# zabaras/deep-turbulence

Measured on AMD Instinct MI355X. Metric: flow-field samples/sec (fwd+log-det+bwd), 64x256x256x4; optimizer step: HipAdam (one-launch Adam, same update as torch.optim.Adam), higher is better.
Workload: dtype f32; 1 GPU; tmglow M: sample()+logdet+backward+Adam, out 256x256x4, L=4, K=16, batch 64/GPU; global_batch=64, parallelism=dp1, world_size_observed=1, rank0_device=AMD Radeon Graphics cuda:0, mix_precision=f32, launch=eager

## Files before the change

### deep-turbulence_amd/csrc/tmg_conv.hip

```cpp
#include "tmg_common.h"
#include <stdlib.h>

static __device__ float g_tmg_zero_page[64];

struct ConvP {
    TmgSeg in[TMG_MAX_IN_SEG];
    int nseg;
    int vec4;
    int B, Hin, Win, Hout, Wout;
    int ksize, stride;
    int Cin, Cin_pad, Cout, Cout_pad;
    const float* wpk;
    const float* bias;
    const float* kappa;
    const float* in_scale;
    const float* in_shift;
    int relu_in, pad_rep, relu_out, accumulate;
    TmgOSeg out[TMG_MAX_OUT_SEG];
    int nout;
    TmgSeg add;
    int TW_log2, TH;
    int KCH;
    int tiles_x, tiles_y;
    int ntiles, nchunks;
    int ovec4;
};

template <int MT, int NTW, int WM, int WN>
__global__ __launch_bounds__(256) void conv_mfma_kernel(ConvP p) {
    extern __shared__ __attribute__((aligned(16))) float lds[];
    const int tid = threadIdx.x, lane = tid & 63, wave = tid >> 6;
    const int wm = wave % WM, wn = wave / WM;
    const int li = lane & 15, q = lane >> 4;
    constexpr int MBLK = 16 * MT * WM;

    int t = blockIdx.x;
    const int tx = t % p.tiles_x;
    t /= p.tiles_x;
    const int ty = t % p.tiles_y;
    const int b = t / p.tiles_y;
    const int TWl = p.TW_log2, TW = 1 << TWl, TH = MBLK >> TWl;
    const int oy0 = ty * TH, ox0 = tx * TW;
    const int s = p.stride, halo = p.ksize >> 1;
    const int PW = s * (TW - 1) + 1 + 2 * halo, PH = s * (TH - 1) + 1 + 2 * halo;
    const int iy0 = s * oy0 - halo, ix0 = s * ox0 - halo;
    const int ntaps = p.ksize * p.ksize;
    const int KB = p.Cin_pad >> 4;

// ... 97 lines not shown
        }
        float* obase = op_ + ooff + nl;
#pragma unroll
        for (int i = 0; i < MT; ++i) {
#pragma unroll
            for (int r = 0; r < 4; ++r) {
                const int m = (wm * MT + i) * 16 + q * 4 + r;
                const int oy = oy0 + (m >> TWl), ox = ox0 + (m & (TW - 1));
                if (oy < p.Hout && ox < p.Wout) {
                    const size_t opx = ((size_t)b * p.Hout + oy) * p.Wout + ox;
                    float v = acc[i][j][r] + bv;
                    if (p.add.p) v += p.add.p[opx * p.add.stride + p.add.off + n];
                    v *= osc;
                    if (p.relu_out) v = fmaxf(v, 0.f);
                    float* dst = obase + opx * ostride;
                    if (p.accumulate) v += *dst;
                    *dst = v;
                }
            }
        }
    }
}

template <int MT, int NTW, int WM, int WN>
__global__ __launch_bounds__(512, 1) void conv_fwd_kernel(ConvP p) {
    extern __shared__ __attribute__((aligned(16))) float lds[];
    constexpr int NT = 512, UP = 7;
    const int tid = threadIdx.x, lane = tid & 63;
    const int wave = __builtin_amdgcn_readfirstlane(tid >> 6);
    const int wm = wave % WM, wn = wave / WM;
    const int li = lane & 15, q = lane >> 4;
    constexpr int MBLK = 16 * MT * WM;
    const int TWl = p.TW_log2, TW = 1 << TWl, TH = MBLK >> TWl;
    const int halo = p.ksize >> 1, ntaps = p.ksize * p.ksize;
    const int PW = TW + 2 * halo, PH = TH + 2 * halo, PHPW = PH * PW;
    const int KB = p.Cin_pad >> 4, KCH = p.KCH, CS = KCH + 8, CS4 = CS >> 2;
    const int bufw = PHPW * CS;
    const int nchunks = p.nchunks;
    const int ntiles_total = p.Cout_pad >> 4;
    const int ntile0 = (blockIdx.y * WN + wn) * NTW;
    const float* zero_page = g_tmg_zero_page;

    f32x4 acc[MT][NTW];
#pragma unroll
    for (int i = 0; i < MT; ++i)
#pragma unroll
        for (int j = 0; j < NTW; ++j) acc[i][j] = (f32x4){0.f, 0.f, 0.f, 0.f};
    int abase[MT], mrc[MT];
// ... 31 lines not shown
    int ti_b = (int)blockIdx.x / tpi, ti_y = ((int)blockIdx.x - ti_b * tpi) / p.tiles_x, ti_x = (int)blockIdx.x - ti_b * tpi - ti_y * p.tiles_x;
    int tm_b = ti_b, tm_y = ti_y, tm_x = ti_x;
#define TMG_FW_ADVANCE(X, Y, B_)                                  \
    {                                                             \
        X += Gx;                                                  \
        if (X >= p.tiles_x) { X -= p.tiles_x; ++Y; }              \
        Y += Gy;                                                  \
        if (Y >= p.tiles_y) { Y -= p.tiles_y; ++B_; }             \
        B_ += Gb;                                                 \
    }
    const float osc = out_scale_of(p.kappa);
    constexpr bool HB = MT * NTW <= 8;
    float4 biasq[HB ? NTW : 1];
    if (HB) {
#pragma unroll
        for (int j = 0; j < NTW; ++j) {
            const int n0 = (ntile0 + j) * 16 + 4 * q;
            float b4[4];
#pragma unroll
            for (int r = 0; r < 4; ++r) b4[r] = (p.bias && n0 + r < p.Cout) ? p.bias[n0 + r] : 0.f;
            biasq[HB ? j : 0] = make_float4(b4[0], b4[1], b4[2], b4[3]);
        }
    }
    float4 b0[NTW], b1[NTW];
    if (nst > 0) {
#pragma unroll
        for (int j = 0; j < NTW; ++j) b0[j] = tmg_bload4(wrs, boff0, TMG_FW_BOFF(j));
    }

    for (int k = -2; k < nst; ++k) {
        if (k >= -1 && k + 1 < nst) {
            const int c0 = cc * KCH, kch = min(KCH, p.Cin_pad - c0);
            const bool pcv = 4 * pc4 < kch;
            float4 isc = make_float4(1.f, 1.f, 1.f, 1.f), ish = make_float4(0.f, 0.f, 0.f, 0.f);
            if (p.in_scale) {
                const int c = c0 + 4 * pc4;
                float* fs = reinterpret_cast<float*>(&isc);
                float* fh = reinterpret_cast<float*>(&ish);
#pragma unroll
                for (int e = 0; e < 4; ++e)
                    if (c + e < p.Cin) { fs[e] = p.in_scale[c + e]; fh[e] = p.in_shift[c + e]; }
            }
            char* bb = reinterpret_cast<char*>(lds) + 4u * (((k + 1) & 1) * bufw) + pdst0;
#pragma unroll
            for (int u = 0; u < UP; ++u) {
                if (pcv && ppix0 + u * pstep < PHPW) {
// ... 24 lines not shown
                        if (cl >= p.in[1].n) {
                            cl -= p.in[1].n;
                            sp = p.in[2].p; ss = p.in[2].stride; so = p.in[2].off;
                        }
                    }
                    tptr = sp + so + cl;
                    tss = ss;
                }
            }
            const int iy0 = oy0_ - halo, ix0 = ox0_ - halo;
            const int tbv = b_ * p.Hin * p.Win * tss;
            oobm = 0;
#pragma unroll
            for (int u = 0; u < UP; ++u) {
                const int iy = iy0 + (int)(pyx[u] >> 16), ix = ix0 + (int)(pyx[u] & 0xffffu);
                const int iyc = min(max(iy, 0), p.Hin - 1), ixc = min(max(ix, 0), p.Win - 1);
                const bool oob = !p.pad_rep && (iy != iyc || ix != ixc);
                const int elem = (int)__umul24(__umul24(iyc, p.Win) + ixc, tss) + tbv;
                const float* a_ = (oob || ppix0 + u * pstep >= PHPW) ? zero_page : tptr + elem;
                pv[u] = *reinterpret_cast<const float4*>(a_);
                if (p.in_scale) oobm |= (oob ? 1u : 0u) << u;
            }
            if (++ci == nchunks) { ci = 0; TMG_FW_ADVANCE(ti_x, ti_y, ti_b) }
        }
        if (k >= 0) {
            const int c0 = cm * KCH, kch = min(KCH, p.Cin_pad - c0);
            const int kbn = kch >> 4, niter = ntaps * kbn;
            const float4* lds4 = reinterpret_cast<const float4*>(lds + (k & 1) * bufw);
            const float* wl = p.wpk + (size_t)(c0 >> 4) * kb_stride;
            const int c0n = (cm + 1 == nchunks) ? 0 : c0 + KCH;
            const float* wl_next = p.wpk + (size_t)(c0n >> 4) * kb_stride;
            int tap = 0, kb = 0, txx = 0;
            constexpr bool PREADD = MT * NTW <= 8;
            float4 addv[PREADD ? MT : 1][PREADD ? NTW : 1];
            if (PREADD && p.add.p && p.ovec4 && cm + 1 == nchunks) {
                const int b_ = tm_b, oy0_ = tm_y * TH, ox0_ = tm_x * TW;
#pragma unroll
                for (int i = 0; i < MT; ++i) {
                    const int oy = min(oy0_ + (mrc[i] >> 16), p.Hout - 1), ox = min(ox0_ + (mrc[i] & 0xffff), p.Wout - 1);
                    const unsigned opx = (unsigned)(__umul24(b_ * p.Hout + oy, p.Wout) + ox);
#pragma unroll
                    for (int j = 0; j < NTW; ++j) {
                        const int n0 = min((ntile0 + j) * 16 + 4 * q, p.Cout - 4);
                        addv[PREADD ? i : 0][PREADD ? j : 0] = *reinterpret_cast<const float4*>(p.add.p + (size_t)opx * (unsigned)p.add.stride + p.add.off + n0);
                    }
                }
// ... 19 lines not shown
                _Pragma("unroll") for (int i = 0; i < MT; ++i) _Pragma("unroll") for (int j = 0; j < NTW; ++j)       \
                    acc[i][j] = __builtin_amdgcn_mfma_f32_16x16x4f32(BC[j].y, af[i].y, acc[i][j], 0, 0, 0);          \
                _Pragma("unroll") for (int i = 0; i < MT; ++i) _Pragma("unroll") for (int j = 0; j < NTW; ++j)       \
                    acc[i][j] = __builtin_amdgcn_mfma_f32_16x16x4f32(BC[j].z, af[i].z, acc[i][j], 0, 0, 0);          \
                _Pragma("unroll") for (int i = 0; i < MT; ++i) _Pragma("unroll") for (int j = 0; j < NTW; ++j)       \
                    acc[i][j] = __builtin_amdgcn_mfma_f32_16x16x4f32(BC[j].w, af[i].w, acc[i][j], 0, 0, 0);          \
            }
            int it = 0;
            for (; it + 1 < niter; it += 2) {
                TMG_FW_BODY(b0, b1)
                TMG_FW_BODY(b1, b0)
            }
            if (it < niter) {
                TMG_FW_BODY(b0, b1)
#pragma unroll
                for (int j = 0; j < NTW; ++j) b0[j] = b1[j];
            }
#undef TMG_FW_BODY
            if (cm + 1 == nchunks) {
                const int b_ = tm_b, oy0_ = tm_y * TH, ox0_ = tm_x * TW;
                int qe = q;
                asm volatile("" : "+v"(qe));
                const bool store_only = p.ovec4 && !p.accumulate && (HB || !p.bias) && (PREADD || !p.add.p);
                if (store_only) {
#pragma unroll
                    for (int i = 0; i < MT; ++i) {
                        const int oy = oy0_ + (mrc[i] >> 16), ox = ox0_ + (mrc[i] & 0xffff);
                        if (oy < p.Hout && ox < p.Wout) {
                            const unsigned opx = (unsigned)(__umul24(b_ * p.Hout + oy, p.Wout) + ox);
#pragma unroll
                            for (int j = 0; j < NTW; ++j) {
                                const int n0 = (ntile0 + j) * 16 + 4 * qe;
                                if (n0 < p.Cout) {
                                    float v[4] = {acc[i][j][0], acc[i][j][1], acc[i][j][2], acc[i][j][3]};
                                    if (HB) { v[0] += biasq[HB ? j : 0].x; v[1] += biasq[HB ? j : 0].y; v[2] += biasq[HB ? j : 0].z; v[3] += biasq[HB ? j : 0].w; }
                                    if (PREADD && p.add.p) {
                                        const float4 a4 = addv[PREADD ? i : 0][PREADD ? j : 0];
                                        v[0] += a4.x; v[1] += a4.y; v[2] += a4.z; v[3] += a4.w;
                                    }
#pragma unroll
                                    for (int r = 0; r < 4; ++r) {
                                        v[r] *= osc;
                                        if (p.relu_out) v[r] = fmaxf(v[r], 0.f);
                                    }
                                    int nl = n0;
                                    TMG_PICK_OSEG(p.out, nl, op_, ostride, ooff)
                                    *reinterpret_cast<float4*>(op_ + (size_t)opx * (unsigned)ostride + ooff + nl) = make_float4(v[0], v[1], v[2], v[3]);
// ... 929 lines not shown
    int l = 0;
    while ((1 << l) < v) ++l;
    return l;
}

static void fill_fwd_plan(int64_t* plan, int kernel, int MT, int NTW, int WM, int WN, const ConvP& p, int gx, int gy, size_t lds_bytes) {
    const int64_t v[16] = {kernel, MT, NTW, WM, WN, p.TW_log2, p.TH, p.tiles_x, p.tiles_y, p.KCH, (p.Cin_pad + p.KCH - 1) / p.KCH, gx, gy,
                           (int64_t)lds_bytes, p.vec4, kernel == 0 ? p.ovec4 : 0};
    for (int i = 0; i < 16; ++i) plan[i] = v[i];
}

template <int MT, int NTW, int WM, int WN>
static int launch_conv(const ConvP& p, int gy, size_t lds_bytes, hipStream_t st, int64_t* plan) {
    if (plan) { fill_fwd_plan(plan, 1, MT, NTW, WM, WN, p, p.B * p.tiles_x * p.tiles_y, gy, lds_bytes); return 0; }
    TMG_LDS_OPTIN((&conv_mfma_kernel<MT, NTW, WM, WN>));
    dim3 grid(p.B * p.tiles_x * p.tiles_y, gy, 1);
    const int kid = (WM == 4 ? NTW - 1 : (WM == 2 ? NTW + 1 : NTW + 3));
    ProfScope prof(kid, 2.0 * p.B * p.Hout * p.Wout * (double)p.Cout * p.Cin * p.ksize * p.ksize, st);
    hipLaunchKernelGGL((conv_mfma_kernel<MT, NTW, WM, WN>), grid, dim3(256), lds_bytes, st, p);
    TMG_CHECK_LAUNCH();
    return 0;
}

template <int MT, int NTW, int WM, int WN>
static int launch_fwd(const ConvP& p, int G, int gy, size_t lds_bytes, hipStream_t st, int64_t* plan) {
    if (plan) { fill_fwd_plan(plan, 0, MT, NTW, WM, WN, p, G, gy, lds_bytes); return 0; }
    TMG_LDS_OPTIN((&conv_fwd_kernel<MT, NTW, WM, WN>));
    const int kid = p.ksize == 1 ? 31 : 11 + (WM == 8 ? NTW - 1 : (WM == 4 ? NTW + 1 : NTW + 3));
    ProfScope prof(kid, 2.0 * p.B * p.Hout * p.Wout * (double)p.Cout * p.Cin * p.ksize * p.ksize, st);
    hipLaunchKernelGGL((conv_fwd_kernel<MT, NTW, WM, WN>), dim3(G, gy, 1), dim3(512), lds_bytes, st, p);
    TMG_CHECK_LAUNCH();
    return 0;
}

static int conv_fwd_lean(ConvP p, hipStream_t st, int64_t* plan) {
    if (p.stride != 1 || !p.vec4 || (p.Cin & 3) || (long)p.Hin * p.Win >= (1 << 24) || (long)p.B * p.Hout >= (1 << 24) ||
        p.Wout >= (1 << 24) || (long)p.B * p.Hout * p.Wout >= (1L << 32))
        return -100;
    for (int i = 0; i < p.nseg; ++i)
        if (p.in[i].stride >= (1 << 24) || (long)p.B * p.Hin * p.Win * p.in[i].stride >= (1L << 31)) return -100;
    p.ovec4 = (p.Cout & 3) == 0;
    for (int i = 0; i < p.nout; ++i)
        if (((p.out[i].stride | p.out[i].off | p.out[i].n) & 3) || (((uintptr_t)p.out[i].p) & 15)) p.ovec4 = 0;
    if (p.add.p && (((p.add.stride | p.add.off) & 3) || (((uintptr_t)p.add.p) & 15))) p.ovec4 = 0;
    const int ntt = p.Cout_pad >> 4;
    int WM, WN, NTW;
    if (ntt <= 4) { WM = 8; WN = 1; NTW = ntt; }
    else if (ntt <= 8) { WM = 4; WN = 2; NTW = ntt <= 6 ? 3 : 4; }
    else { WM = 2; WN = 4; NTW = ntt <= 12 ? 3 : 4; }
    const int gy = (ntt + WN * NTW - 1) / (WN * NTW);
    const long npix = (long)p.B * p.Hout * p.Wout;
    const int halo = p.ksize >> 1;
    for (int MT = 4; MT >= 1; MT >>= 1) {
        if (MT > 1 && (npix / (16 * MT * WM)) * gy < 256) continue;
        const int MBLK = 16 * MT * WM;
        int twl = ilog2_ceil(p.Wout);
        if (twl > 5) twl = 5;
        if (twl < 2) twl = 2;
        while ((1 << twl) > MBLK) --twl;
        while (twl < 5 && (MBLK >> twl) > p.Hout && (1 << twl) < p.Wout) ++twl;
        const int TW = 1 << twl, TH = MBLK >> twl;
        if (TH < 1) continue;
        const int PHPW = (TW + 2 * halo) * (TH + 2 * halo);
        int nchunks = (p.Cin_pad + 63) / 64, kch = 0;
        for (; nchunks <= p.Cin_pad / 16; ++nchunks) {
            kch = (((p.Cin_pad / 16) + nchunks - 1) / nchunks) * 16;
            const int k4p = kch <= 16 ? 4 : (kch <= 32 ? 8 : 16);
            if (PHPW * k4p <= 7 * 512 && 2 * (size_t)PHPW * (kch + 8) * 4 <= 160 * 1024) break;
            kch = 0;
        }
        if (!kch) continue;
        p.TW_log2 = twl; p.TH = TH;
        p.tiles_x = (p.Wout + TW - 1) / TW;
        p.tiles_y = (p.Hout + TH - 1) / TH;
        p.ntiles = p.B * p.tiles_x * p.tiles_y;
        p.KCH = kch;
        p.nchunks = (p.Cin_pad + kch - 1) / kch;
        const int G = tmg_persistent_grid(gy, p.ntiles);
        const size_t lds_bytes = 2 * (size_t)PHPW * (kch + 8) * 4;
#define TMG_FWD_CASE(NTW_, WM_, WN_)                                                                   \
        if (NTW == NTW_ && WM == WM_ && WN == WN_) {                                                   \
            if (MT == 4) return launch_fwd<4, NTW_, WM_, WN_>(p, G, gy, lds_bytes, st, plan);                \
            if (MT == 2) return launch_fwd<2, NTW_, WM_, WN_>(p, G, gy, lds_bytes, st, plan);                \
            return launch_fwd<1, NTW_, WM_, WN_>(p, G, gy, lds_bytes, st, plan);                             \
        }
        TMG_FWD_CASE(1, 8, 1) TMG_FWD_CASE(2, 8, 1) TMG_FWD_CASE(3, 8, 1) TMG_FWD_CASE(4, 8, 1)
        TMG_FWD_CASE(3, 4, 2) TMG_FWD_CASE(4, 4, 2) TMG_FWD_CASE(3, 2, 4) TMG_FWD_CASE(4, 2, 4)
        TMG_FWD_CASE(2, 4, 2) TMG_FWD_CASE(1, 4, 2) TMG_FWD_CASE(2, 2, 4) TMG_FWD_CASE(1, 2, 4)
#undef TMG_FWD_CASE
        return -100;
    }
    return -100;
}

extern "C" int tmg_conv_pack_map(const void* w, void* wpk, int64_t Cout, int64_t Cin, int64_t cin_eff, int64_t ksize, int64_t mode,
                                 const int64_t* map, hipStream_t st);

extern "C" int tmg_conv_pack(const void* w, void* wpk, int64_t Cout, int64_t Cin, int64_t cin_eff, int64_t ksize, int64_t mode,
                             hipStream_t st) {
    const int64_t map[3] = {Cin, 0x7fffffff, 0};
    return tmg_conv_pack_map(w, wpk, Cout, Cin, cin_eff < Cin ? Cin : cin_eff, ksize, mode, map, st);
}
// ... 136 lines not shown
    TMG_CONV_CASE(4, 2, 2)
    TMG_CONV_CASE(3, 1, 4)
    TMG_CONV_CASE(4, 1, 4)
#undef TMG_CONV_CASE
    return -7;
}

extern "C" int tmg_conv_fwd_add(const void* const* in_ptrs, const int64_t* in_desc, int64_t nseg, const void* wpk, const void* bias,
                                const void* kappa, const void* in_scale, const void* in_shift, const void* add,
                                const int64_t* add_desc, void* const* out_ptrs, const int64_t* out_desc, int64_t nout,
                                const int64_t* dims, hipStream_t st) {
    return conv_fwd_impl(in_ptrs, in_desc, nseg, wpk, bias, kappa, in_scale, in_shift, add, add_desc, out_ptrs, out_desc, nout, dims, st,
                         nullptr);
}

extern "C" int tmg_conv_fwd_plan(const void* const* in_ptrs, const int64_t* in_desc, int64_t nseg, const void* wpk, const void* bias,
                                 const void* kappa, const void* in_scale, const void* in_shift, const void* add,
                                 const int64_t* add_desc, void* const* out_ptrs, const int64_t* out_desc, int64_t nout,
                                 const int64_t* dims, hipStream_t st, int64_t* plan) {
    if (!plan) return -3;
    for (int i = 0; i < 16; ++i) plan[i] = -1;
    return conv_fwd_impl(in_ptrs, in_desc, nseg, wpk, bias, kappa, in_scale, in_shift, add, add_desc, out_ptrs, out_desc, nout, dims, st,
                         plan);
}

template <int NP, int NCO, bool LEAN>
static int launch_wgrad(const WgradP& p, dim3 grid, size_t lds_bytes, hipStream_t st, int64_t* plan, size_t ws_floats) {
    if (plan) {
        const int64_t v[15] = {NP, NCO, LEAN ? 1 : 0, p.ksplit, p.MPIX, p.TH, p.TW_log2, p.CITG, p.PPG, grid.x, grid.y, grid.z, p.ws ? 1 : 0,
                               (int64_t)lds_bytes, (int64_t)ws_floats};
        for (int i = 0; i < 15; ++i) plan[i] = v[i];
        return 0;
    }
    TMG_LDS_OPTIN((&conv_wgrad_kernel<NP, NCO, LEAN>));
    const int nco_i = NCO == 1 ? 0 : (NCO == 2 ? 1 : 2);
    const int kid = NP == 3 ? 8 + nco_i : (NP == 8 ? 28 + nco_i : 19 + ((NP - 5) / 2) * 3 + nco_i);
    const double ngr = p.gtab ? (double)(grid.y / (p.bpg > 0 ? p.bpg : 1)) : 1.0;
    ProfScope prof(kid, ngr * 2.0 * p.B * p.Hout * p.Wout * (double)p.Cout * p.Cin * p.ksize * p.ksize, st);
    hipLaunchKernelGGL((conv_wgrad_kernel<NP, NCO, LEAN>), grid, dim3(512), lds_bytes, st, p);
    TMG_CHECK_LAUNCH();
    return 0;
}

struct WgradPlan {
    int twl, TH, MPIX, tiles_x, tiles_y, ntiles, CITG, PPG, NCO, NP, ksplit, gx, gy, gz;
    size_t lds_bytes, ws_floats;
// ... 293 lines not shown
```

### deep-turbulence_amd/tmg_hip.py

```python
import ctypes
import os
import weakref
import subprocess
import sys

import torch

_HERE = os.path.dirname(os.path.abspath(__file__))
LIB_PATH = os.path.join(_HERE, "libtmglow_hip.so")
CSRC = os.path.join(_HERE, "csrc")
SOURCES = ["tmg_conv.hip", "tmg_pointwise.hip", "tmg_physics.hip", "tmg_mix16.hip", "tmg_coupling.hip", "tmg_wino.hip", "tmg_thin.hip", "tmg_glue.hip", "tmg_ensemble.hip", "tmg_spectrum.hip", "tmg_scores.hip"]
NO_PACKED_F32 = ["tmg_wino.hip", "tmg_conv.hip", "tmg_coupling.hip", "tmg_thin.hip", "tmg_mix16.hip", "tmg_spectrum.hip"]
_lib = None

c_i64 = ctypes.c_int64
c_vp = ctypes.c_void_p

EXPORTS = [
    "tmg_conv_pack", "tmg_conv_pack_map", "tmg_conv_fwd", "tmg_conv_fwd_add", "tmg_affine_bwd_scaled", "tmg_c1_fwd_add", "tmg_conv_wgrad", "tmg_conv_wgrad_ws_floats", "tmg_conv_rep_border_fix", "tmg_conv_dgrad_direct",
    "tmg_affine_apply", "tmg_affine_apply_pass", "tmg_bn_finalize", "tmg_affine_bwd", "tmg_lstm_pointwise_fwd", "tmg_lstm_pointwise_bwd", "tmg_gauss_fwd",
    "tmg_gauss_bwd", "tmg_checker", "tmg_upsample_fwd", "tmg_upsample_bwd", "tmg_chan_reduce", "tmg_bn_bwd_apply",
    "tmg_phys_fwd", "tmg_phys_rms", "tmg_phys_bwd", "tmg_conv_wgrad_grouped", "tmg_conv_wgrad_grouped_ws_floats", "tmg_conv_pack_batched", "tmg_masked_add", "tmg_c1x2_fwd", "tmg_c1_fwd", "tmg_c1_bwd", "tmg_dense2_bwd", "tmg_dkappa", "tmg_prof_enable", "tmg_prof_collect", "tmg_mix_f16", "tmg_phys_bwd_dev", "tmg_coupling_fwd", "tmg_coupling_bwd",
    "tmg_conv_wino_pack", "tmg_conv_wino_fwd", "tmg_conv_wino_narrow", "tmg_conv_wino_wgrad", "tmg_conv_wino_wgrad_ws_floats", "tmg_mix_f32", "tmg_lu_fold_fwd", "tmg_lu_fold_bwd", "tmg_lu_fold_bwd_split", "tmg_level_finish", "tmg_conv_wgrad_thin_grouped", "tmg_mix_wgrad_grouped", "tmg_layer_planes", "tmg_conv_wino_wgrad_grouped", "tmg_conv_wino_wgrad_grouped_ws_floats", "tmg_adam_step", "tmg_chan_moments", "tmg_bn_finalize64", "tmg_mix_f32_affine_fwd", "tmg_mix_f32_affine_bwd", "tmg_conv_pack_many", "tmg_pad_halves", "tmg_coupling_fwd_halves", "tmg_coupling_bwd_halves", "tmg_fill_i64", "tmg_conv_wino_pack3", "tmg_conv_wino_fwd3", "tmg_mat_inverse", "tmg_gauss_sample", "tmg_reverse_loss_fwd", "tmg_reverse_loss_bwd", "tmg_sum_terms", "tmg_vec_sum", "tmg_level_pack", "tmg_spread2", "tmg_phys_fields", "tmg_phys_fields_bwd",
    "tmg_gauss_sample_keyed", "tmg_ens_accum", "tmg_ens_time_finalize", "tmg_ens_turb_accum", "tmg_ens_turb_finalize",
    "tmg_spec_rows", "tmg_spec_cols", "tmg_spec_accum", "tmg_spec_finalize",
    "tmg_ens_score_store", "tmg_ens_score_step",
]
PLAN_EXPORTS = ["tmg_conv_fwd_plan", "tmg_conv_wgrad_plan", "tmg_conv_rep_border_plan"]
RET_I64 = ("tmg_conv_wgrad_ws_floats", "tmg_conv_wgrad_grouped_ws_floats", "tmg_conv_wino_wgrad_ws_floats",
           "tmg_conv_wino_wgrad_grouped_ws_floats")


def build(force=False, verbose=False):
    from concurrent.futures import ThreadPoolExecutor
    inc = os.path.join(os.path.dirname(_HERE), "include")
    headers = [os.path.join(CSRC, "tmg_common.h"), os.path.join(inc, "tmglow_hip.h"), os.path.join(inc, "tmglow_hip_plan.h")]
    hmt = max(os.path.getmtime(h) for h in headers)
    objdir = os.path.join(_HERE, "build")
    os.makedirs(objdir, exist_ok=True)
    hipcc = os.environ.get("HIPCC", "/opt/rocm/bin/hipcc")
    flags = ["--offload-arch=gfx950", "-O3", "-fPIC", "-std=c++17", "-Wno-unused-result", "-I", inc]
    jobs, objs, stamps = [], [], []
    for src in SOURCES:
        sp, ob = os.path.join(CSRC, src), os.path.join(objdir, src.replace(".hip", ".o"))
        objs.append(ob)
        extra = ["-Xclang", "-target-feature", "-Xclang", "-packed-fp32-ops"] if src in NO_PACKED_F32 else []
        line = " ".join(flags + extra)
        stamp = ob + ".flags"
        old = open(stamp).read() if os.path.exists(stamp) else None
        if force or old != line or not os.path.exists(ob) or os.path.getmtime(ob) < max(os.path.getmtime(sp), hmt):
            jobs.append([hipcc] + flags + extra + ["-c", sp, "-o", ob])
# ... 8 lines not shown
        err = "\n".join(ln for ln in r.stderr.splitlines() if "'-packed-fp32-ops' is not a recognized feature" not in ln)
        if err.strip():
            print(err, file=sys.stderr, flush=True)
        if r.returncode != 0:
            raise subprocess.CalledProcessError(r.returncode, cmd)

    with ThreadPoolExecutor(max_workers=4) as ex:
        list(ex.map(run, jobs))
    for stamp, line in stamps:
        open(stamp, "w").write(line)
    run([hipcc, "--offload-arch=gfx950", "-shared", "-fPIC"] + objs + ["-o", LIB_PATH])
    return LIB_PATH


def lib():
    global _lib
    if _lib is None:
        if not os.path.exists(LIB_PATH):
            raise RuntimeError("libtmglow_hip.so is missing (%s): run `python -c 'import __graft_entry__ as g; g.build()'`. "
                               "There is no fallback path." % LIB_PATH)
        _lib = ctypes.CDLL(LIB_PATH)
        for name in EXPORTS:
            getattr(_lib, name).restype = c_i64 if name in RET_I64 else ctypes.c_int
        _lib.tmg_prof_name.restype = ctypes.c_char_p
        for name in PLAN_EXPORTS:
            getattr(_lib, name).restype = ctypes.c_int
            getattr(_lib, name).argtypes = PLAN_ARGTYPES[name]
    return _lib


def prof_enable(on):
    lib().tmg_prof_enable(c_i64(int(on)))


def prof_kernel_id(name):
    l = lib()
    for k in range(64):
        if l.tmg_prof_name(c_i64(k)).decode() == name:
            return k
    raise KeyError(name)


def prof_collect():
    l = lib()
    nk = 64
    buf = (ctypes.c_double * (3 * nk))()
# ... 515 lines not shown


def adam_step(tab, chunks, nchunks, lr, b1, b2, eps, wd, bc1, bc2s, amsgrad):
    _chk(lib().tmg_adam_step(_ptr(tab), _ptr(chunks), _i64(nchunks, 1 if amsgrad else 0), _flts([lr, b1, b2, eps, wd, bc1, bc2s, 1.0 - b1, 1.0 - b2]), _stream()),
         "tmg_adam_step")


def mix_f32(x, W, bias, y, transposed=False):
    B, Hh, Ww, C = x.shape
    if C > 128 or C % 4:
        return False
    _chk(lib().tmg_mix_f32(_ptr(x), _d2(x), _ptr(W), _ptr(bias), _ptr(y), _d2(y), _i64(B * Hh * Ww, C, 1 if transposed else 0), _stream()),
         "tmg_mix_f32")
    return True


def mix_affine_fwd(x, hh, W, bias, y, r, y2, logdet):
    B, Hh, Ww, C = x.shape
    rc = lib().tmg_mix_f32_affine_fwd(_ptr(x), _d2(x), _ptr(hh), _d2(hh), _ptr(W), _ptr(bias), _ptr(y), _d2(y), _ptr(r), _ptr(y2),
                                      _ptr(logdet), _i64(B * Hh * Ww, C, Hh * Ww), _stream())
    return _launched(rc, "tmg_mix_f32_affine_fwd")


def mix_affine_bwd(dy, W, r, t2, g, kappa, dto1, dtin2, dhh):
    B, Hh, Ww, C = dy.shape
    rc = lib().tmg_mix_f32_affine_bwd(_ptr(dy), _d2(dy), _ptr(W), _ptr(r), _ptr(t2), _d2(t2), _ptr(g), _ptr(kappa), _ptr(dto1), _ptr(dtin2),
                                      _d2(dtin2), _ptr(dhh), _d2(dhh), _i64(B * Hh * Ww, C, Hh * Ww), _stream())
    return _launched(rc, "tmg_mix_f32_affine_bwd")


def conv_rep_border_fix(dy, w, outs, kappa=None):
    B, H, W, Cdy = dy.shape
    op, odesc, n_out = _segs(outs)
    Cx = sum(t.shape[3] for t in outs)
    _chk(lib().tmg_conv_rep_border_fix(_ptr(dy), _d2(dy), _ptr(w), _ptr(kappa), op, odesc, c_i64(n_out), _i64(B, H, W, Cdy, Cx),
                                       _stream()), "tmg_conv_rep_border_fix")


FWD_PLAN_FIELDS = ("kernel", "MT", "NTW", "WM", "WN", "TW_log2", "TH", "tiles_x", "tiles_y", "KCH", "nchunks", "grid_x", "grid_y",
                   "lds_bytes", "vec4", "ovec4")
WGRAD_PLAN_FIELDS = ("NP", "NCO", "LEAN", "ksplit", "MPIX", "TH", "TW_log2", "CITG", "PPG", "gx", "gy", "gz", "slab", "lds_bytes",
                     "ws_floats")
BORDER_PLAN_FIELDS = ("mfma", "NT", "S", "tiles", "blocks")
PLAN_ARGTYPES = {
    "tmg_conv_fwd_plan": [c_vp, c_vp, c_i64, c_vp, c_vp, c_vp, c_vp, c_vp, c_vp, c_vp, c_vp, c_vp, c_i64, c_vp, c_vp, c_vp],
    "tmg_conv_wgrad_plan": [c_vp, c_vp, c_i64, c_vp, c_vp, c_vp, c_vp, c_vp, c_vp, c_vp, c_vp, c_i64, c_vp, c_vp, c_i64, c_vp],
    "tmg_conv_rep_border_plan": [c_vp, c_vp, c_vp, c_vp, c_vp, c_vp, c_i64, c_vp, c_vp, c_vp],
}


def _pseg(t):
    if isinstance(t, torch.Tensor):
        B, H, W, C = t.shape
        d = seg(t)
        return (B, H, W), d[0], d[1], d[3]
    shp, addr, stride, n = t
    return tuple(shp), int(addr), int(stride), int(n)


def _psegs(ts):
    d = [_pseg(t) for t in ts]
    return (c_vp * len(d))(*[x[1] for x in d]), (c_i64 * (3 * len(d)))(*[v for x in d for v in (x[2], 0, x[3])]), len(d), d


def _pp(t):
    if t is None or t is False:
        return c_vp(0)
    if isinstance(t, torch.Tensor):
        return c_vp(t.data_ptr())
    if isinstance(t, tuple):
# ... 367 lines not shown
```

### deep-turbulence_amd/tmg_ops.py

```python
import collections
import math

import os
import threading
import weakref

import torch

import tmg_hip as H

LOG5 = math.log(5.0)
LOG4 = math.log(4.0)
SPLIT_LIMITS = (-2.0, LOG5, -2.0, LOG5)
TOP_LIMITS = (0.0, 0.0, -10.0, LOG5)


class _ZeroPool:
    CHUNK = 8 << 20
    LIMIT = 2 << 20

    def __init__(self):
        self.lock = threading.Lock()
        self.cur = {}

# ... 980 lines not shown
            out = empty(bhw + (C,), dev)
        r = empty(bhw + (ch,), dev)
        y2 = empty(bhw + (ch,), dev) if reverse else None
        ok = H.coupling_fwd(tin, out, r, y2, D, Hc[..., k * C:(k + 1) * C], L.wzs[k], L.bzs[k], L.kps[k], Wm[k] if reverse else None,
                            bm[k] if reverse else None, logdet, reverse, L.cin)
        assert ok
        if L.rec:
            return out, None
        return out, ((tin, D, r, [t1, y2]) if reverse else (tin, D, r, out, cur))

    @staticmethod
    def _fwd_wide(L, k, cur, Wm, bm, PM, PZ, Hc, dc_of, logdet, mixaff):
        C, ch, reverse = L.C, L.ch, L.reverse
        bhw, dev = Hc.shape[:3], Hc.device
        tin = cur if reverse else _mix_fwd(cur, Wm[k], bm[k], PM[k])
        x1 = tin[..., :ch]
        if ch % 4 == 0:
            D = LevelCouplingFn._growth(L, k, x1, dc_of)
        else:
            D = empty(bhw + (4,), dev)
            add1, add2 = dc_of(k)
            H.c1_fwd([x1], L.w1s[k], D[..., 0:1], relu_in=True, w_rows=ch, fill4=True, add=add1)
            H.c1_fwd([x1, D], L.w2s[k], D[..., 1:2], relu_in=True, w_rows=ch + 1, w_split=ch, w_gap=L.Cc, add=add2)
        hh = empty(bhw + (C,), dev)
        H.conv_fwd([x1, D], PZ[k], C, 3, 1, [hh], bias=L.bzs[k], kappa=L.kps[k], relu_in=True, pad_rep=True, add=Hc[..., k * C:(k + 1) * C])
        r = empty(bhw + (ch,), dev)
        if mixaff:
            y2 = empty(bhw + (ch,), dev)
            out = empty(bhw + (C,), dev)
            if H.mix_affine_fwd(tin, hh, Wm[k], bm[k], out, r, y2, logdet):
                return out, (tin, D, r, [x1, y2])
        y = empty(bhw + (C,), dev)
        H.affine_apply(hh, tin[..., ch:], y[..., ch:], r, logdet, reverse, x1=x1, y1=y[..., :ch])
        return (_mix_fwd(y, Wm[k], bm[k], PM[k]) if reverse else y), (tin, D, r, y) + (() if reverse else (cur,))

    @staticmethod
    def forward(ctx, x, cond, Wm, bm, reverse, *wts):
        x = x if x.stride(3) == 1 else x.contiguous()
        cond = cond.contiguous()
        L = _level(wts, x.shape[3], cond.shape[3], reverse)
        NL, C, ch = L.NL, L.C, L.ch
        dev = x.device
        Wz, Wcat, Bz, Kp = LevelCouplingFn._level_operands(L, dev)
        Hc, Dc, dc_of = LevelCouplingFn._cond_parts(L, cond, Wcat)
        logdet = zeros(x.shape[0], dev)
        PZ = H.conv_pack_batched(Wz, 0, ch + 4, (ch + 2, ch, L.Cc))
        PM = H.conv_pack_batched(Wm.reshape(NL, C, C, 1, 1), 0)
        mixaff = (reverse and C in (64, 128) and Wm.is_contiguous() and bm.is_contiguous()
                  and os.environ.get("TMG_NO_MIX_AFFINE") is None)
# ... 573 lines not shown
```

### include/tmglow_hip.h

```cpp
#ifndef TMGLOW_HIP_H
#define TMGLOW_HIP_H
#include <stdint.h>

#ifdef __cplusplus
extern "C" {
#endif

#ifndef TMG_MAX_IN_SEG
#define TMG_MAX_IN_SEG 3
#define TMG_MAX_OUT_SEG 3
#endif

typedef struct ihipStream_t* tmg_stream_t;


int tmg_conv_pack(const void* w, void* wpk, int64_t Cout, int64_t Cin, int64_t cin_eff, int64_t ksize, int64_t mode,
                  tmg_stream_t st);

int tmg_conv_pack_map(const void* w, void* wpk, int64_t Cout, int64_t Cin, int64_t cin_eff, int64_t ksize, int64_t mode,
                      const int64_t* map, tmg_stream_t st);

int tmg_conv_fwd(const void* const* in_ptrs, const int64_t* in_desc, int64_t nseg, const void* wpk, const void* bias,
                 const void* kappa, const void* in_scale, const void* in_shift, void* const* out_ptrs,
                 const int64_t* out_desc, int64_t nout, const int64_t* dims, tmg_stream_t st);
// ... 138 lines not shown
int tmg_lu_fold_bwd(const void* tab, const void* sign_s, const void* perm, const void* iperm, const void* W, const void* dWm, const void* dbm,
                    const void* dld, void* dl, void* du, void* dlogs, void* da, void* db, const int64_t* dims, const float* fl, tmg_stream_t st);
int tmg_lu_fold_bwd_split(const void* tab, const void* sign_s, const void* perm, const void* iperm, const void* W, const void* dWm,
                          const void* dbm, const void* dWm_tail, const void* dbm_tail, const void* dld, void* dl, void* du, void* dlogs,
                          void* da, void* db, const int64_t* dims, const float* fl, tmg_stream_t st);

int tmg_conv_wgrad_thin_grouped(const void* gtab, int64_t G, const int64_t* seg_channels, int64_t nseg, const void* dy, int64_t dy_stride,
                                void* dW, const int64_t* dims, tmg_stream_t st);

int tmg_mix_wgrad_grouped(const void* gtab, int64_t G, void* dW, void* db, const int64_t* dims, tmg_stream_t st);

int tmg_layer_planes(const void* src, void* dst, int64_t npix, int64_t CP, tmg_stream_t st);

int tmg_level_finish(const void* Wz, const void* dWz, const void* Bz, const void* dBz, const void* Kp, const void* tmpX, const void* tmpC,
                     void* dW1, void* dW2, void* dK, void* ws, const int64_t* dims, tmg_stream_t st);

int tmg_mix_f32(const void* x, const int64_t* x_d, const void* W, const void* bias, void* y, const int64_t* y_d,
                const int64_t* dims, tmg_stream_t st);
int tmg_mix_f32_affine_fwd(const void* x, const int64_t* x_d, const void* hh, const int64_t* hh_d, const void* W, const void* bias,
                           void* y, const int64_t* y_d, void* r, void* y2, void* logdet, const int64_t* dims, tmg_stream_t st);
int tmg_mix_f32_affine_bwd(const void* dy, const int64_t* dy_d, const void* W, const void* r, const void* t2, const int64_t* t2_d,
                           const void* g, const void* kappa, void* dto1, void* dtin2, const int64_t* dtin2_d, void* dhh,
                           const int64_t* dhh_d, const int64_t* dims, tmg_stream_t st);


#define TMG_SUM_TERMS_MAX 8

int tmg_gauss_sample(const void* hz, const int64_t* hz_d, const void* eps_in, const int64_t* ei_d, const void* pass,
                     const int64_t* p_d, void* out, const int64_t* o_d, int64_t pass_off, void* eps_out, void* logp, const void* nonce,
                     const int64_t* dims, const float* fl, tmg_stream_t st);
int tmg_gauss_sample_keyed(const void* hz, const int64_t* hz_d, const void* eps_in, const int64_t* ei_d, const void* pass,
                           const int64_t* p_d, void* out, const int64_t* o_d, int64_t pass_off, void* eps_out, void* logp,
                           const void* keys, const int64_t* dims, const float* fl, tmg_stream_t st);

int tmg_ens_accum(const void* y, const int64_t* y_d, const void* u, const void* out_mu, const void* out_std, void* smean, void* sm2,
                  void* tmean, void* tm2, void* mean_out, void* std_out, void* mag_mean, void* mag_std, const int64_t* o_d,
                  const int64_t* dims, tmg_stream_t st);
int tmg_ens_time_finalize(const void* tmean, const void* tm2, void* tm_mean, void* tm_std, void* rms_mean, void* rms_std,
                          const int64_t* dims, tmg_stream_t st);
int tmg_ens_turb_accum(const void* y, const int64_t* y_d, const void* u, const void* out_mu, const void* out_std, const void* tmean,
                       void* vmean, void* vm2, void* cuv, void* tvort, void* vort_mean, void* vort_std, const int64_t* dims,
                       const float* fl, tmg_stream_t st);
int tmg_ens_turb_finalize(const void* tm2, const void* cuv, const void* tvort, void* uv_mean, void* uv_std, void* tke_mean,
                          void* tke_std, void* tv_mean, void* tv_std, const int64_t* dims, tmg_stream_t st);

int tmg_ens_score_store(const void* y, const int64_t* y_d, void* xs, const int64_t* dims, tmg_stream_t st);
// ... 39 lines not shown
```

### include/tmglow_hip_plan.h

```cpp
#ifndef TMGLOW_HIP_PLAN_H
#define TMGLOW_HIP_PLAN_H

int tmg_conv_fwd_plan(const void* const* in_ptrs, const int64_t* in_desc, int64_t nseg, const void* wpk, const void* bias,
                      const void* kappa, const void* in_scale, const void* in_shift, const void* add, const int64_t* add_desc,
                      void* const* out_ptrs, const int64_t* out_desc, int64_t nout, const int64_t* dims, tmg_stream_t st,
                      int64_t* plan);
int tmg_conv_wgrad_plan(const void* const* in_ptrs, const int64_t* in_desc, int64_t nseg, const void* in_scale,
                        const void* in_shift, const void* dy, const int64_t* dy_desc, void* dW, void* dbias, const void* kappa,
                        void* ws, int64_t ws_floats, const int64_t* dims, tmg_stream_t st, int64_t ngroups, int64_t* plan);
int tmg_conv_rep_border_plan(const void* dy, const int64_t* dy_desc, const void* w, const void* kappa, void* const* out_ptrs,
                             const int64_t* out_desc, int64_t nout, const int64_t* dims, tmg_stream_t st, int64_t* plan);

#endif
```

Measured before the change: 1487 samples/s.

## Fuse coupling 3x3 conv with affine transform and 1x1 mix in one kernel

Adds a CPL variant of the forward conv kernel whose epilogue applies the affine coupling (softsign scale, exp, shift, log-det accumulation) and then the channel-mixing 1x1 matmul via MFMA, with the mix weights staged in LDS. The intermediate hh tensor is no longer written to and re-read from global memory, and one launch per coupling step is saved. In exchange it needs extra LDS (lowering tile and chunk options), adds a __syncthreads exchange between waves when WN=2, raises register pressure in the epilogue, and uses atomics for logdet. It falls back to the old path when its shape constraints fail.

New measurement: 1513 samples/s (median of 5 runs). +1.7%, better.

```diff
diff --git a/deep-turbulence_amd/csrc/tmg_conv.hip b/deep-turbulence_amd/csrc/tmg_conv.hip
--- a/deep-turbulence_amd/csrc/tmg_conv.hip
+++ b/deep-turbulence_amd/csrc/tmg_conv.hip
@@ -24,6 +24,11 @@
     int tiles_x, tiles_y;
     int ntiles, nchunks;
     int ovec4;
+    const float* cx; int cxs;
+    const float* cW; const float* cb;
+    float* cy; int cys;
+    float* cr; float* cy2;
+    float* cld;
 };
 
 template <int MT, int NTW, int WM, int WN>
@@ -167,8 +172,128 @@
     }
 }
 
-template <int MT, int NTW, int WM, int WN>
+template <int WN>
+__device__ __forceinline__ void cplw_stage_w(const float* __restrict__ W, const float* __restrict__ bias, float4* Wl, int tid) {
+    constexpr int C = 64 * WN, ch = C / 2, NU = C * C / 4 / 512;
+    float2 wa[NU], wb[NU];
+    const float4 bq = tmg_ldg4(bias + 4 * (tid & (C / 4 - 1)));
+#pragma unroll
+    for (int u = 0; u < NU; ++u) {
+        const int idx = tid + u * 512, kq = idx / C, co = idx - kq * C;
+        const int t = kq - ch / 4;
+        const int ca = t < 0 ? 4 * kq : ch + 16 * (t >> 2) + 2 * (t & 3), cb = t < 0 ? ca + 2 : ca + 8;
+        wa[u] = tmg_ldg2(W + (size_t)co * C + ca);
+        wb[u] = tmg_ldg2(W + (size_t)co * C + cb);
+    }
+#pragma unroll
+    for (int u = 0; u < NU; ++u) Wl[tid + u * 512] = make_float4(wa[u].x, wa[u].y, wb[u].x, wb[u].y);
+    if (tid < C / 4) Wl[C * C / 4 + tid] = bq;
+}
+
+template <int MT, int WM, int WN>
+__device__ __forceinline__ void cplw_epilogue(const ConvP& p, f32x4 (&acc)[MT][4], const float4 (&biasq)[4], const float4 (&addv)[MT][4],
+                                              const float4* Wl, float4* Xl, float osc,
+                                              const int (&mrc)[MT], int b_, int oy0_, int ox0_, int li, int q, int wm, int wn, int lane) {
+    static_assert(WN == 1 || MT == 1, "the y2 exchange buffer holds one m-tile per wave");
+    constexpr int C = 64 * WN, ch = C / 2, HT = 2 * WN;
+    const bool has_add = p.add.p != nullptr;
+    float ldsum = 0.f;
+#pragma unroll
+    for (int i = 0; i < MT; ++i)
+#pragma unroll
+        for (int j = 0; j < 4; ++j) {
+            float v[4] = {acc[i][j][0], acc[i][j][1], acc[i][j][2], acc[i][j][3]};
+            v[0] += biasq[j].x; v[1] += biasq[j].y; v[2] += biasq[j].z; v[3] += biasq[j].w;
+            if (has_add) { v[0] += addv[i][j].x; v[1] += addv[i][j].y; v[2] += addv[i][j].z; v[3] += addv[i][j].w; }
+            acc[i][j] = (f32x4){v[0] * osc, v[1] * osc, v[2] * osc, v[3] * osc};
+        }
+    float2 x2v[MT][4];
+#pragma unroll
+    for (int i = 0; i < MT; ++i) {
+        const int oy = min(oy0_ + (mrc[i] >> 16), p.Hout - 1), ox = min(ox0_ + (mrc[i] & 0xffff), p.Wout - 1);
+        const unsigned opx = (unsigned)(__umul24(b_ * p.Hout + oy, p.Wout) + ox);
+#pragma unroll
+        for (int j = 0; j < 4; ++j) x2v[i][j] = tmg_ldg2(p.cx + (size_t)opx * (unsigned)p.cxs + ch + 8 * (wn * 4 + j) + 2 * q);
+    }
+#pragma unroll
+    for (int i = 0; i < MT; ++i) {
+        const int oy = oy0_ + (mrc[i] >> 16), ox = ox0_ + (mrc[i] & 0xffff);
+        const bool ok = oy < p.Hout && ox < p.Wout;
+        const unsigned opx = (unsigned)(__umul24(b_ * p.Hout + min(oy, p.Hout - 1), p.Wout) + min(ox, p.Wout - 1));
+        const float* xb = p.cx + (size_t)opx * (unsigned)p.cxs;
+        float4 x1v[HT];
+#pragma unroll
+        for (int ks = 0; ks < HT; ++ks) x1v[ks] = tmg_ldg4(xb + 16 * ks + 4 * q);
+        float4 yq[2];
+        float* const rb = p.cr + (size_t)opx * ch + wn * 32 + 2 * q;
+#pragma unroll
+        for (int j = 0; j < 4; ++j) {
+            const float sh[2] = {acc[i][j][0], acc[i][j][2]}, rr[2] = {acc[i][j][1], acc[i][j][3]}, xx[2] = {x2v[i][j].x, x2v[i][j].y};
+            float oo[2];
+#pragma unroll
+            for (int e = 0; e < 2; ++e) {
+                const float sg = 2.f * rr[e] / (1.f + fabsf(rr[e]));
+                oo[e] = xx[e] * expf(-sg) - sh[e];
+                ldsum += ok ? sg : 0.f;
+            }
+            float* yf = reinterpret_cast<float*>(&yq[j >> 1]) + 2 * (j & 1);
+            yf[0] = oo[0]; yf[1] = oo[1];
+            if (ok) *reinterpret_cast<float2*>(rb + 8 * j) = make_float2(rr[0], rr[1]);
+        }
+        float4 yo[2];
+        if (WN == 2) {
+            Xl[((wn * WM + wm) * 2 + 0) * 64 + lane] = yq[0];
+            Xl[((wn * WM + wm) * 2 + 1) * 64 + lane] = yq[1];
+            __syncthreads();
+            yo[0] = Xl[(((wn ^ 1) * WM + wm) * 2 + 0) * 64 + lane];
+            yo[1] = Xl[(((wn ^ 1) * WM + wm) * 2 + 1) * 64 + lane];
+        }
+        f32x4 o[4];
+#pragma unroll
+        for (int mt = 0; mt < 4; ++mt) {
+            const float4 cb = Wl[C * C / 4 + (wn * 4 + mt) * 4 + q];
+            o[mt] = (f32x4){cb.x, cb.y, cb.z, cb.w};
+        }
+        const float4* wl = Wl + q * C + wn * 64 + li;
+#define TMG_CW_STEP(KQ, BV)                                                                                                    \
+        {                                                                                                                      \
+            float4 a[4];                                                                                                       \
+            _Pragma("unroll") for (int mt = 0; mt < 4; ++mt) a[mt] = wl[(KQ) * C + mt * 16];                                   \
+            const float4 bq_ = BV;                                                                                             \
+            _Pragma("unroll") for (int mt = 0; mt < 4; ++mt) o[mt] = __builtin_amdgcn_mfma_f32_16x16x4f32(a[mt].x, bq_.x, o[mt], 0, 0, 0); \
+            _Pragma("unroll") for (int mt = 0; mt < 4; ++mt) o[mt] = __builtin_amdgcn_mfma_f32_16x16x4f32(a[mt].y, bq_.y, o[mt], 0, 0, 0); \
+            _Pragma("unroll") for (int mt = 0; mt < 4; ++mt) o[mt] = __builtin_amdgcn_mfma_f32_16x16x4f32(a[mt].z, bq_.z, o[mt], 0, 0, 0); \
+            _Pragma("unroll") for (int mt = 0; mt < 4; ++mt) o[mt] = __builtin_amdgcn_mfma_f32_16x16x4f32(a[mt].w, bq_.w, o[mt], 0, 0, 0); \
+            __builtin_amdgcn_sched_barrier(0);    \
+        }
+#pragma unroll
+        for (int ks = 0; ks < HT; ++ks) TMG_CW_STEP(4 * ks, x1v[ks])
+#pragma unroll
+        for (int h = 0; h < 2; ++h) TMG_CW_STEP(4 * (HT + 2 * wn + h), yq[h])
+        if (WN == 2) {
+#pragma unroll
+            for (int h = 0; h < 2; ++h) TMG_CW_STEP(4 * (HT + 2 * (wn ^ 1) + h), yo[h])
+        }
+#undef TMG_CW_STEP
+        if (ok) {
+            float* yb = p.cy2 + (size_t)opx * ch + wn * 32 + 2 * q;
+#pragma unroll
+            for (int j = 0; j < 4; ++j) {
+                const float* yf = reinterpret_cast<const float*>(&yq[j >> 1]) + 2 * (j & 1);
+                *reinterpret_cast<float2*>(yb + 8 * j) = make_float2(yf[0], yf[1]);
+            }
+            float* ob = p.cy + (size_t)opx * (unsigned)p.cys + wn * 64 + 4 * q;
+#pragma unroll
+            for (int mt = 0; mt < 4; ++mt) *reinterpret_cast<float4*>(ob + 16 * mt) = make_float4(o[mt][0], o[mt][1], o[mt][2], o[mt][3]);
+        }
+    }
+    ldsum = wave_sum(ldsum);
+    if (lane == 0) atomicAdd(p.cld + b_, ldsum);
+}
+
+template <int MT, int NTW, int WM, int WN, int CPL = 0>
 __global__ __launch_bounds__(512, 1) void conv_fwd_kernel(ConvP p) {
+    static_assert(CPL == 0 || (NTW == 4 && WN <= 2 && MT * NTW <= 8), "the coupling epilogue: all of C = 64 WN channels in one block row");
     extern __shared__ __attribute__((aligned(16))) float lds[];
     constexpr int NT = 512, UP = 7;
     const int tid = threadIdx.x, lane = tid & 63;
@@ -246,6 +371,8 @@
             biasq[HB ? j : 0] = make_float4(b4[0], b4[1], b4[2], b4[3]);
         }
     }
+    float4* const cWl = reinterpret_cast<float4*>(lds + 2 * bufw);
+    float4* const cXl = cWl + 16 * WN * 64 * WN + 16 * WN;
     float4 b0[NTW], b1[NTW];
     if (nst > 0) {
 #pragma unroll
@@ -316,6 +443,9 @@
                 if (p.in_scale) oobm |= (oob ? 1u : 0u) << u;
             }
             if (++ci == nchunks) { ci = 0; TMG_FW_ADVANCE(ti_x, ti_y, ti_b) }
+        }
+        if constexpr (CPL != 0) {
+            if (k == -2) cplw_stage_w<WN>(p.cW, p.cb, cWl, tid);
         }
         if (k >= 0) {
             const int c0 = cm * KCH, kch = min(KCH, p.Cin_pad - c0);
@@ -381,7 +511,9 @@
                 int qe = q;
                 asm volatile("" : "+v"(qe));
                 const bool store_only = p.ovec4 && !p.accumulate && (HB || !p.bias) && (PREADD || !p.add.p);
-                if (store_only) {
+                if constexpr (CPL != 0) {
+                    cplw_epilogue<MT, WM, WN>(p, acc, biasq, addv, cWl, cXl, osc, mrc, b_, oy0_, ox0_, li, qe, wm, wn, lane);
+                } else if (store_only) {
 #pragma unroll
                     for (int i = 0; i < MT; ++i) {
                         const int oy = oy0_ + (mrc[i] >> 16), ox = ox0_ + (mrc[i] & 0xffff);
@@ -1357,18 +1489,18 @@
     return 0;
 }
 
-template <int MT, int NTW, int WM, int WN>
+template <int MT, int NTW, int WM, int WN, int CPL = 0>
 static int launch_fwd(const ConvP& p, int G, int gy, size_t lds_bytes, hipStream_t st, int64_t* plan) {
     if (plan) { fill_fwd_plan(plan, 0, MT, NTW, WM, WN, p, G, gy, lds_bytes); return 0; }
-    TMG_LDS_OPTIN((&conv_fwd_kernel<MT, NTW, WM, WN>));
+    TMG_LDS_OPTIN((&conv_fwd_kernel<MT, NTW, WM, WN, CPL>));
     const int kid = p.ksize == 1 ? 31 : 11 + (WM == 8 ? NTW - 1 : (WM == 4 ? NTW + 1 : NTW + 3));
     ProfScope prof(kid, 2.0 * p.B * p.Hout * p.Wout * (double)p.Cout * p.Cin * p.ksize * p.ksize, st);
-    hipLaunchKernelGGL((conv_fwd_kernel<MT, NTW, WM, WN>), dim3(G, gy, 1), dim3(512), lds_bytes, st, p);
+    hipLaunchKernelGGL((conv_fwd_kernel<MT, NTW, WM, WN, CPL>), dim3(G, gy, 1), dim3(512), lds_bytes, st, p);
     TMG_CHECK_LAUNCH();
     return 0;
 }
 
-static int conv_fwd_lean(ConvP p, hipStream_t st, int64_t* plan) {
+static int conv_fwd_lean(ConvP p, hipStream_t st, int64_t* plan, bool cpl = false) {
     if (p.stride != 1 || !p.vec4 || (p.Cin & 3) || (long)p.Hin * p.Win >= (1 << 24) || (long)p.B * p.Hout >= (1 << 24) ||
         p.Wout >= (1 << 24) || (long)p.B * p.Hout * p.Wout >= (1L << 32))
         return -100;
@@ -1386,7 +1518,10 @@
     const int gy = (ntt + WN * NTW - 1) / (WN * NTW);
     const long npix = (long)p.B * p.Hout * p.Wout;
     const int halo = p.ksize >> 1;
+    const size_t lds_extra = cpl ? (size_t)p.Cout * p.Cout * 4 + (size_t)p.Cout * 4 + (WN == 2 ? 8 * 2 * 64 * 16 : 0) : 0;
+    if (cpl && (!p.ovec4 || NTW != 4 || gy != 1)) return -100;
     for (int MT = 4; MT >= 1; MT >>= 1) {
+        if (cpl && MT * WN > 2) continue;
         if (MT > 1 && (npix / (16 * MT * WM)) * gy < 256) continue;
         const int MBLK = 16 * MT * WM;
         int twl = ilog2_ceil(p.Wout);
@@ -1401,7 +1536,7 @@
         for (; nchunks <= p.Cin_pad / 16; ++nchunks) {
             kch = (((p.Cin_pad / 16) + nchunks - 1) / nchunks) * 16;
             const int k4p = kch <= 16 ? 4 : (kch <= 32 ? 8 : 16);
-            if (PHPW * k4p <= 7 * 512 && 2 * (size_t)PHPW * (kch + 8) * 4 <= 160 * 1024) break;
+            if (PHPW * k4p <= 7 * 512 && 2 * (size_t)PHPW * (kch + 8) * 4 + lds_extra <= 160 * 1024) break;
             kch = 0;
         }
         if (!kch) continue;
@@ -1412,7 +1547,11 @@
         p.KCH = kch;
         p.nchunks = (p.Cin_pad + kch - 1) / kch;
         const int G = tmg_persistent_grid(gy, p.ntiles);
-        const size_t lds_bytes = 2 * (size_t)PHPW * (kch + 8) * 4;
+        const size_t lds_bytes = 2 * (size_t)PHPW * (kch + 8) * 4 + lds_extra;
+        if (cpl) {
+            if (WN == 1) return MT == 2 ? launch_fwd<2, 4, 8, 1, 1>(p, G, gy, lds_bytes, st, plan) : launch_fwd<1, 4, 8, 1, 1>(p, G, gy, lds_bytes, st, plan);
+            return launch_fwd<1, 4, 4, 2, 1>(p, G, gy, lds_bytes, st, plan);
+        }
 #define TMG_FWD_CASE(NTW_, WM_, WN_)                                                                   \
         if (NTW == NTW_ && WM == WM_ && WN == WN_) {                                                   \
             if (MT == 4) return launch_fwd<4, NTW_, WM_, WN_>(p, G, gy, lds_bytes, st, plan);                \
@@ -1595,6 +1734,49 @@
     for (int i = 0; i < 16; ++i) plan[i] = -1;
     return conv_fwd_impl(in_ptrs, in_desc, nseg, wpk, bias, kappa, in_scale, in_shift, add, add_desc, out_ptrs, out_desc, nout, dims, st,
                          plan);
+}
+
+static int coupling_wide_impl(const void* x, const int64_t* x_d, const void* d, const int64_t* d_d, const void* wpk, const void* bz,
+                              const void* kappa, const void* add, const int64_t* add_d, const void* W, const void* bias, void* y,
+                              const int64_t* y_d, void* r, void* y2, void* logdet, const int64_t* dims, hipStream_t st, int64_t* plan) {
+    const int C = (int)dims[3], ch = C / 2;
+    if ((C != 64 && C != 128) || dims[4] != 0 || dims[0] <= 0 || dims[1] <= 0 || dims[2] <= 0) return -100;
+    const TmgD2 ad = tmg_opt_d2(add, add_d);
+    if (((x_d[0] | x_d[1] | d_d[0] | d_d[1] | y_d[0] | y_d[1] | ad.stride | ad.off) & 3) || x_d[0] < C || y_d[0] < C || d_d[0] < 4) return -100;
+    if ((((uintptr_t)x) | ((uintptr_t)d) | ((uintptr_t)add) | ((uintptr_t)W) | ((uintptr_t)bias) | ((uintptr_t)y) | ((uintptr_t)r) | ((uintptr_t)y2)) & 15)
+        return -100;
+    if (!x || !d || !wpk || !W || !bias || !y || !r || !y2 || !logdet) return -100;
+    ConvP p = {};
+    p.in[0] = TmgSeg{(const float*)x, (int)x_d[0], (int)x_d[1], ch};
+    p.in[1] = TmgSeg{(const float*)d, (int)d_d[0], (int)d_d[1], 4};
+    p.nseg = 2; p.vec4 = 1;
+    p.B = (int)dims[0]; p.Hin = p.Hout = (int)dims[1]; p.Win = p.Wout = (int)dims[2];
+    p.ksize = 3; p.stride = 1; p.Cin = ch + 4; p.Cout = C;
+    p.Cin_pad = (p.Cin + 15) & ~15; p.Cout_pad = C;
+    p.relu_in = 1; p.pad_rep = 1;
+    p.wpk = (const float*)wpk; p.bias = (const float*)bz; p.kappa = (const float*)kappa;
+    p.add = TmgSeg{(const float*)add, ad.stride, ad.off, 0};
+    p.out[0] = TmgOSeg{(float*)y, (int)y_d[0], (int)y_d[1], C}; p.nout = 1;
+    p.cx = (const float*)x + x_d[1]; p.cxs = (int)x_d[0];
+    p.cW = (const float*)W; p.cb = (const float*)bias;
+    p.cy = (float*)y + y_d[1]; p.cys = (int)y_d[0];
+    p.cr = (float*)r; p.cy2 = (float*)y2; p.cld = (float*)logdet;
+    return conv_fwd_lean(p, st, plan, true);
+}
+
+extern "C" int tmg_coupling_wide_fwd(const void* x, const int64_t* x_d, const void* d, const int64_t* d_d, const void* wpk, const void* bz,
+                                     const void* kappa, const void* add, const int64_t* add_d, const void* W, const void* bias, void* y,
+                                     const int64_t* y_d, void* r, void* y2, void* logdet, const int64_t* dims, hipStream_t st) {
+    return coupling_wide_impl(x, x_d, d, d_d, wpk, bz, kappa, add, add_d, W, bias, y, y_d, r, y2, logdet, dims, st, nullptr);
+}
+
+extern "C" int tmg_coupling_wide_fwd_plan(const void* x, const int64_t* x_d, const void* d, const int64_t* d_d, const void* wpk, const void* bz,
+                                          const void* kappa, const void* add, const int64_t* add_d, const void* W, const void* bias, void* y,
+                                          const int64_t* y_d, void* r, void* y2, void* logdet, const int64_t* dims, hipStream_t st,
+                                          int64_t* plan) {
+    if (!plan) return -3;
+    for (int i = 0; i < 16; ++i) plan[i] = -1;
+    return coupling_wide_impl(x, x_d, d, d_d, wpk, bz, kappa, add, add_d, W, bias, y, y_d, r, y2, logdet, dims, st, plan);
 }
 
 template <int NP, int NCO, bool LEAN>
diff --git a/deep-turbulence_amd/tmg_hip.py b/deep-turbulence_amd/tmg_hip.py
--- a/deep-turbulence_amd/tmg_hip.py
+++ b/deep-turbulence_amd/tmg_hip.py
@@ -26,7 +26,8 @@
     "tmg_spec_rows", "tmg_spec_cols", "tmg_spec_accum", "tmg_spec_finalize",
     "tmg_ens_score_store", "tmg_ens_score_step",
 ]
-PLAN_EXPORTS = ["tmg_conv_fwd_plan", "tmg_conv_wgrad_plan", "tmg_conv_rep_border_plan"]
+PLAN_EXPORTS = ["tmg_conv_fwd_plan", "tmg_conv_wgrad_plan", "tmg_conv_rep_border_plan", "tmg_coupling_wide_fwd_plan"]
+WIDE_EXPORTS = ["tmg_coupling_wide_fwd"]
 RET_I64 = ("tmg_conv_wgrad_ws_floats", "tmg_conv_wgrad_grouped_ws_floats", "tmg_conv_wino_wgrad_ws_floats",
            "tmg_conv_wino_wgrad_grouped_ws_floats")
 
@@ -81,6 +82,8 @@
         _lib = ctypes.CDLL(LIB_PATH)
         for name in EXPORTS:
             getattr(_lib, name).restype = c_i64 if name in RET_I64 else ctypes.c_int
+        for name in WIDE_EXPORTS:
+            getattr(_lib, name).restype = ctypes.c_int
         _lib.tmg_prof_name.restype = ctypes.c_char_p
         for name in PLAN_EXPORTS:
             getattr(_lib, name).restype = ctypes.c_int
@@ -642,6 +645,24 @@
     return _launched(rc, "tmg_mix_f32_affine_fwd")
 
 
+def coupling_wide_fwd(x, D, wpk, bz, kappa, add, W, bias, y, r, y2, logdet, mix_f16=False):
+    B, Hh, Ww, C = x.shape
+    rc = lib().tmg_coupling_wide_fwd(_ptr(x), _d2(x), _ptr(D), _d2(D), _ptr(wpk), _ptr(bz), _ptr(kappa), _ptr(add), _d2(add), _ptr(W),
+                                     _ptr(bias), _ptr(y), _d2(y), _ptr(r), _ptr(y2), _ptr(logdet), _i64(B, Hh, Ww, C, 1 if mix_f16 else 0),
+                                     _stream())
+    return _launched(rc, "tmg_coupling_wide_fwd")
+
+
+def coupling_wide_fwd_plan(x, D, add, y, C, mix_f16=False):
+    (B, Hh, Ww), xp, xs, _ = _pseg(x)
+    _, dp, ds, _ = _pseg(D)
+    _, yp, ys, _ = _pseg(y)
+    ap, as_ = (_pseg(add)[1], _pseg(add)[2]) if add is not None else (0, 0)
+    return _plan_call("tmg_coupling_wide_fwd_plan", FWD_PLAN_FIELDS, c_vp(xp), _i64(xs, 0), c_vp(dp), _i64(ds, 0), c_vp(16), c_vp(16), c_vp(16),
+                      c_vp(ap), _i64(as_, 0), c_vp(16), c_vp(16), c_vp(yp), _i64(ys, 0), c_vp(16), c_vp(16), c_vp(16),
+                      _i64(B, Hh, Ww, C, 1 if mix_f16 else 0), None)
+
+
 def mix_affine_bwd(dy, W, r, t2, g, kappa, dto1, dtin2, dhh):
     B, Hh, Ww, C = dy.shape
     rc = lib().tmg_mix_f32_affine_bwd(_ptr(dy), _d2(dy), _ptr(W), _ptr(r), _ptr(t2), _d2(t2), _ptr(g), _ptr(kappa), _ptr(dto1), _ptr(dtin2),
@@ -666,6 +687,7 @@
     "tmg_conv_fwd_plan": [c_vp, c_vp, c_i64, c_vp, c_vp, c_vp, c_vp, c_vp, c_vp, c_vp, c_vp, c_vp, c_i64, c_vp, c_vp, c_vp],
     "tmg_conv_wgrad_plan": [c_vp, c_vp, c_i64, c_vp, c_vp, c_vp, c_vp, c_vp, c_vp, c_vp, c_vp, c_i64, c_vp, c_vp, c_i64, c_vp],
     "tmg_conv_rep_border_plan": [c_vp, c_vp, c_vp, c_vp, c_vp, c_vp, c_i64, c_vp, c_vp, c_vp],
+    "tmg_coupling_wide_fwd_plan": [c_vp] * 19,
 }
 
 
diff --git a/deep-turbulence_amd/tmg_ops.py b/deep-turbulence_amd/tmg_ops.py
--- a/deep-turbulence_amd/tmg_ops.py
+++ b/deep-turbulence_amd/tmg_ops.py
@@ -1026,9 +1026,15 @@
             add1, add2 = dc_of(k)
             H.c1_fwd([x1], L.w1s[k], D[..., 0:1], relu_in=True, w_rows=ch, fill4=True, add=add1)
             H.c1_fwd([x1, D], L.w2s[k], D[..., 1:2], relu_in=True, w_rows=ch + 1, w_split=ch, w_gap=L.Cc, add=add2)
+        r = empty(bhw + (ch,), dev)
+        if mixaff and os.environ.get("TMG_NO_WIDE_FUSED") is None:
+            y2 = empty(bhw + (ch,), dev)
+            out = empty(bhw + (C,), dev)
+            if H.coupling_wide_fwd(tin, D, PZ[k], L.bzs[k], L.kps[k], Hc[..., k * C:(k + 1) * C], Wm[k], bm[k], out, r, y2, logdet,
+                                   mix_f16=_MIX_PRECISION == "f16"):
+                return out, (tin, D, r, [x1, y2])
         hh = empty(bhw + (C,), dev)
         H.conv_fwd([x1, D], PZ[k], C, 3, 1, [hh], bias=L.bzs[k], kappa=L.kps[k], relu_in=True, pad_rep=True, add=Hc[..., k * C:(k + 1) * C])
-        r = empty(bhw + (ch,), dev)
         if mixaff:
             y2 = empty(bhw + (ch,), dev)
             out = empty(bhw + (C,), dev)
diff --git a/include/tmglow_hip.h b/include/tmglow_hip.h
--- a/include/tmglow_hip.h
+++ b/include/tmglow_hip.h
@@ -184,6 +184,7 @@
 int tmg_mix_f32_affine_bwd(const void* dy, const int64_t* dy_d, const void* W, const void* r, const void* t2, const int64_t* t2_d,
                            const void* g, const void* kappa, void* dto1, void* dtin2, const int64_t* dtin2_d, void* dhh,
                            const int64_t* dhh_d, const int64_t* dims, tmg_stream_t st);
+#include "tmglow_hip_wide.h"
 
 
 #define TMG_SUM_TERMS_MAX 8
diff --git a/include/tmglow_hip_plan.h b/include/tmglow_hip_plan.h
--- a/include/tmglow_hip_plan.h
+++ b/include/tmglow_hip_plan.h
@@ -10,5 +10,9 @@
                         void* ws, int64_t ws_floats, const int64_t* dims, tmg_stream_t st, int64_t ngroups, int64_t* plan);
 int tmg_conv_rep_border_plan(const void* dy, const int64_t* dy_desc, const void* w, const void* kappa, void* const* out_ptrs,
                              const int64_t* out_desc, int64_t nout, const int64_t* dims, tmg_stream_t st, int64_t* plan);
+int tmg_coupling_wide_fwd_plan(const void* x, const int64_t* x_d, const void* d, const int64_t* d_d, const void* wpk, const void* bz,
+                               const void* kappa, const void* add, const int64_t* add_d, const void* W, const void* bias, void* y,
+                               const int64_t* y_d, void* r, void* y2, void* logdet, const int64_t* dims, tmg_stream_t st,
+                               int64_t* plan);
 
 #endif
diff --git a/include/tmglow_hip_wide.h b/include/tmglow_hip_wide.h
--- /dev/null
+++ b/include/tmglow_hip_wide.h
@@ -0,0 +1,8 @@
+#ifndef TMGLOW_HIP_WIDE_H
+#define TMGLOW_HIP_WIDE_H
+
+int tmg_coupling_wide_fwd(const void* x, const int64_t* x_d, const void* d, const int64_t* d_d, const void* wpk, const void* bz,
+                          const void* kappa, const void* add, const int64_t* add_d, const void* W, const void* bias, void* y,
+                          const int64_t* y_d, void* r, void* y2, void* logdet, const int64_t* dims, tmg_stream_t st);
+
+#endif
```
